# lior1990/hp-vae-gan

Measured on AMD Instinct MI355X. Metric: train iters/sec per pyramid scale, air_balloons 13f@144p, higher is better.
Workload: dtype f32

## Files before the change

### hp-vae-gan_amd/csrc/conv_mfma.hip

```cpp
#include "hpvg_common.h"
#include "hpvg_host.h"
#include "hpvg.h"
#include <stdlib.h>

namespace {

__device__ const float g_zero_word[16] = {0.f, 0.f, 0.f, 0.f, 0.f, 0.f, 0.f, 0.f, 0.f, 0.f, 0.f, 0.f, 0.f, 0.f, 0.f, 0.f};
constexpr long HPVG_ZERO_PLANE_FLOATS = 1L << 18;
__device__ float g_zero_plane[HPVG_ZERO_PLANE_FLOATS];

#ifdef HPVG_TRACE
__device__ unsigned long long g_trace[8192 * 4];
__device__ unsigned long long g_phase[8192 * 4];
#define HPVG_PH(i) { unsigned long long now_ = __builtin_readcyclecounter(); ph_a[i] += now_ - ph_t; ph_t = now_; }
#define HPVG_PH_INIT unsigned long long ph_t = __builtin_readcyclecounter(); unsigned long long ph_a[4] = {0, 0, 0, 0};
#define HPVG_PH_END if (threadIdx.x == 0) { for (int i_ = 0; i_ < 4; ++i_) g_phase[4 * blockIdx.x + i_] = ph_a[i_]; }
#define HPVG_TRACE_BEGIN unsigned long long tr_t0 = wall_clock64(); unsigned long long tr_c0 = __builtin_readcyclecounter();
#define HPVG_TRACE_END                                                              \
  if (threadIdx.x == 0 && blockIdx.x + gridDim.x * (blockIdx.y + gridDim.y * blockIdx.z) < 8192) { \
    unsigned long long* tr = g_trace + 4 * (blockIdx.x + gridDim.x * (blockIdx.y + gridDim.y * blockIdx.z)); \
    tr[0] = tr_t0;                                                                  \
    tr[1] = wall_clock64();                                                         \
    tr[2] = __builtin_amdgcn_s_getreg((31 << 11) | 4);                              \
    tr[3] = (__builtin_amdgcn_s_getreg((31 << 11) | 20) & 0xF) | ((__builtin_readcyclecounter() - tr_c0) << 8); \
// ... 844 lines not shown
          for (int dh = 0; dh < 3; ++dh)
#pragma unroll
            for (int dw = 0; dw < 3; ++dw) {
              const int gwt = gw + dw - 1;
              if (gwt >= 0 && gwt < a.W) v += Pp[(dt * 9 + dh * 3 + dw) * pitch + dh * RS + (dw - 1)];
            }
          sdt[dt] = v;
        }
        rC[p][o] = sdt[0];
        rB[p][o] += sdt[1];
        rA[p][o] += sdt[2];
      }
      __syncthreads();
    }
    if (t >= 1) store_plane(rA, t - 1);
#pragma unroll
    for (int p = 0; p < PPT; ++p)
#pragma unroll
      for (int o = 0; o < COUT; ++o) { rA[p][o] = rB[p][o]; rB[p][o] = rC[p][o]; }
  }
  store_plane(rA, a.T - 1);
}

__global__ void conv_pack_narrow_kernel(const float* __restrict__ w, const float* __restrict__ inv_scale, float* __restrict__ wn,
                                        int Cin_k, int Cout_k, int KT, int NT, int ksteps, int transpose_flip, long total) {
  const long idx = (long)blockIdx.x * blockDim.x + threadIdx.x;
  if (idx >= total) return;
  const int lane = idx & 63;
  long r = idx >> 6;
  const int nt = r % NT;
  const int s = (int)(r / NT);
  const int k = (lane >> 5) * ksteps + s;
  const int n = nt * 32 + (lane & 31);
  const int c = k / KT, dt = k - c * KT;
  const int o = n / 9, tap = dt * 9 + (n - o * 9);
  const int taps = KT * 9;
  float val = 0.f;
  if (o < Cout_k && c < Cin_k) {
    if (!transpose_flip) val = w[((long)o * Cin_k + c) * taps + tap];
    else val = w[((long)c * Cout_k + o) * taps + (taps - 1 - tap)];
    if (inv_scale) val *= inv_scale[0];
  }
  wn[idx] = val;
}

__global__ void conv_pack_kernel(const float* __restrict__ w, const float* __restrict__ inv_scale, float* __restrict__ wp,
                                 int Cin_k, int Cout_k, int taps, int CC, int nchunk, int mbtot, int transpose_flip,
                                 long total_direct, long total) {
  const long idx = (long)blockIdx.x * blockDim.x + threadIdx.x;
  if (idx >= total) return;
  if (idx >= total_direct) {
    const long iw = idx - total_direct;
    const long nw1 = ((long)((Cin_k + WINO_CC - 1) / WINO_CC) * (taps / 9) * 3 * 4 + 4) * mbtot * 64 * (WINO_CC / 2);
    float val = iw < nw1 ? wino_pack_value(w, iw, Cin_k, Cout_k, taps / 9, (Cin_k + WINO_CC - 1) / WINO_CC, mbtot, transpose_flip)
                         : wino2_pack_value(w, iw - nw1, Cin_k, Cout_k, (Cin_k + 3) / 4, 2 * ((mbtot + 1) / 2), transpose_flip);
    if (inv_scale) val *= inv_scale[0];
    wp[idx] = val;
    return;
  }
  const int CP = CC / 2;
  long r = idx;
  const int cp = r % CP; r /= CP;
  const int lane = r % 64; r /= 64;
  const int mb = r % mbtot; r /= mbtot;
  const int tap = r % taps; r /= taps;
  const int ch = (int)r;
  float val = 0.f;
  if (ch < nchunk) {
    const int o = mb * 32 + (lane & 31);
    const int c = ch * CC + 2 * cp + (lane >> 5);
    if (o < Cout_k && c < Cin_k) {
      if (!transpose_flip) val = w[((long)o * Cin_k + c) * taps + tap];
      else val = w[((long)c * Cout_k + o) * taps + (taps - 1 - tap)];
      if (inv_scale) val *= inv_scale[0];
    }
  }
  wp[idx] = val;
}

struct PackBatchArgs {
  const float* w[HPVG_PACK_BATCH_MAX];
  float* wp[HPVG_PACK_BATCH_MAX];
  int flip[HPVG_PACK_BATCH_MAX];
};
__global__ void conv_pack_batch_kernel(const PackBatchArgs a, int C, int taps, int CC, int nchunk, int mbtot, long total_direct,
                                       long total) {
  const long idx = (long)blockIdx.x * blockDim.x + threadIdx.x;
  if (idx >= total) return;
  const int it = blockIdx.y;
  const float* __restrict__ w = a.w[it];
  const int transpose_flip = a.flip[it];
  if (idx >= total_direct) {
    const long iw = idx - total_direct;
    const long nw1 = ((long)((C + WINO_CC - 1) / WINO_CC) * (taps / 9) * 3 * 4 + 4) * mbtot * 64 * (WINO_CC / 2);
    a.wp[it][idx] = iw < nw1 ? wino_pack_value(w, iw, C, C, taps / 9, (C + WINO_CC - 1) / WINO_CC, mbtot, transpose_flip)
                             : wino2_pack_value(w, iw - nw1, C, C, (C + 3) / 4, 2 * ((mbtot + 1) / 2), transpose_flip);
    return;
  }
  const int CP = CC / 2;
  long r = idx;
  const int cp = r % CP; r /= CP;
  const int lane = r % 64; r /= 64;
  const int mb = r % mbtot; r /= mbtot;
  const int tap = r % taps; r /= taps;
  const int ch = (int)r;
  float val = 0.f;
  if (ch < nchunk) {
    const int o = mb * 32 + (lane & 31);
    const int c = ch * CC + 2 * cp + (lane >> 5);
    if (o < C && c < C) {
      if (!transpose_flip) val = w[((long)o * C + c) * taps + tap];
      else val = w[((long)c * C + o) * taps + (taps - 1 - tap)];
    }
  }
  a.wp[it][idx] = val;
}

struct CShape { int B, Cin, Cout, T, H, W, KT; };
inline int conv_check(const CShape& c) {
  if (c.B < 1 || c.Cin < 1 || c.Cout < 1 || c.T < 1 || c.H < 1 || c.W < 1) return HPVG_ERR_ARG;
  return c.KT == 1 || c.KT == 3 ? HPVG_OK : HPVG_ERR_UNSUPPORTED;
}

struct CKnobs {
  bool sk_off;
  bool narrow2_off;
  int narrowt;
  bool w2r;
  bool w2d_off;
  bool w2_split_off;
  int stagger;
  int only_nb, only_mb, only_ntw;
  int env_wino;
  int wino;
  long min_pos;
  int stg;
  int w2d;
  int gen;
// ... 642 lines not shown
    return hpvg_launch_status();
  }
  const int CC = conv_cc(Cin_k);
  hipLaunchKernelGGL(conv_pack_kernel, dim3(hpvg_cdiv(total, 256)), dim3(256), 0, (hipStream_t)stream, w, inv_scale, wp, Cin_k, Cout_k,
                     KT * 9, CC, hpvg_cdiv(Cin_k, CC), hpvg_cdiv(Cout_k, 32), transpose_flip, (long)direct_pack_floats(Cin_k, Cout_k, KT),
                     total);
  return hpvg_launch_status();
}

int pack_batch_launch(int n, const float* const* w, float* const* wp, const int* flip, int C, int KT, bool with2d, void* stream) {
  if (n < 1 || n > HPVG_PACK_BATCH_MAX || !w || !wp || !flip || C <= 4 || (KT != 1 && KT != 3)) return HPVG_ERR_ARG;
  PackBatchArgs a;
  for (int i = 0; i < n; ++i) {
    if (!w[i] || !wp[i]) return HPVG_ERR_ARG;
    a.w[i] = w[i]; a.wp[i] = wp[i]; a.flip[i] = flip[i];
  }
  const int CC = conv_cc(C);
  const long total = (long)wpack_floats(C, C, KT, with2d);
  hipLaunchKernelGGL(conv_pack_batch_kernel, dim3(hpvg_cdiv(total, 256), n), dim3(256), 0, (hipStream_t)stream, a, C, KT * 9, CC,
                     hpvg_cdiv(C, CC), hpvg_cdiv(C, 32), (long)direct_pack_floats(C, C, KT), total);
  return hpvg_launch_status();
}

int write_plan(const Plan& p, int out4, int ntiles, int* out) {
  out[0] = p.L; out[1] = p.Tw; out[2] = p.nrange; out[3] = p.ntw; out[4] = out4; out[5] = p.NB; out[6] = p.MB;
  out[7] = p.gridy; out[8] = (int)p.lds; out[9] = ntiles;
  return HPVG_OK;
}

}

extern "C" {

size_t hpvg_conv_wpack_floats(int Cin, int Cout, int KT) { return wpack_floats(Cin, Cout, KT, true); }
size_t hpvg_conv_wpack_floats_for(int Cin, int Cout, int KT, int B, int T, int H, int W) {
  return wpack_floats(Cin, Cout, KT, wants_wino2d({B, Cin, Cout, T, H, W, KT}));
}
int hpvg_conv_wants_wino2d(int B, int Cin, int Cout, int T, int H, int W, int KT) { return wants_wino2d({B, Cin, Cout, T, H, W, KT}) ? 1 : 0; }

int hpvg_conv_pack_weight_f32(const float* w, const float* inv_scale, float* wp, int Cin_layer, int Cout_layer, int KT,
                              int transpose_flip, void* stream) {
  return pack_weight_launch(w, inv_scale, wp, Cin_layer, Cout_layer, KT, transpose_flip, true, stream);
}
int hpvg_conv_pack_weight_for_f32(const float* w, const float* inv_scale, float* wp, int Cin_layer, int Cout_layer, int KT,
                                  int transpose_flip, int B, int T, int H, int W, void* stream) {
  const int Cin_k = transpose_flip ? Cout_layer : Cin_layer, Cout_k = transpose_flip ? Cin_layer : Cout_layer;
  return pack_weight_launch(w, inv_scale, wp, Cin_layer, Cout_layer, KT, transpose_flip, wants_wino2d({B, Cin_k, Cout_k, T, H, W, KT}), stream);
}
int hpvg_conv_pack_weight_batch_f32(int n, const float* const* w, float* const* wp, const int* flip, int C, int KT, void* stream) {
  return pack_batch_launch(n, w, wp, flip, C, KT, true, stream);
}
int hpvg_conv_pack_weight_batch_for_f32(int n, const float* const* w, float* const* wp, const int* flip, int C, int KT, int B, int T,
                                        int H, int W, void* stream) {
  return pack_batch_launch(n, w, wp, flip, C, KT, wants_wino2d({B, C, C, T, H, W, KT}), stream);
}

int hpvg_conv_fwd_f32(const float* x, const float* wp, const float* bias, const float* in_scale, const float* in_shift,
                      int in_lrelu, float* y, int out_lrelu, const float* out_mask, void* ws, size_t ws_bytes, int B, int Cin,
                      int Cout, int T, int H, int W, int KT, void* stream) {
  return conv_fwd_launch({x, wp, bias, in_scale, in_shift, in_lrelu, y, out_lrelu, out_mask, nullptr, nullptr, ws, ws_bytes,
                          {B, Cin, Cout, T, H, W, KT}, (hipStream_t)stream});
}

size_t hpvg_conv_mask_words(int B, int C, int T, int H, int W) { return (size_t)B * T * H * W * hpvg_cdiv(C, 32); }

int hpvg_conv_fwd_bits_f32(const float* x, const float* wp, const float* bias, float* y, int out_lrelu, const unsigned* mask_bits,
                           unsigned* bits_out, void* ws, size_t ws_bytes, int B, int Cin, int Cout, int T, int H, int W, int KT,
                           void* stream) {
  if (conv_is_narrow(Cin, Cout)) return HPVG_ERR_UNSUPPORTED;
  if (mask_bits && bits_out) return HPVG_ERR_UNSUPPORTED;
  return conv_fwd_launch({x, wp, bias, nullptr, nullptr, 0, y, out_lrelu, nullptr, mask_bits, bits_out, ws, ws_bytes,
                          {B, Cin, Cout, T, H, W, KT}, (hipStream_t)stream});
}

int hpvg_conv_fwd_kernel_kind(int B, int Cin, int Cout, int T, int H, int W, int KT) {
  const CShape c{B, Cin, Cout, T, H, W, KT};
  return conv_check(c) == HPVG_OK ? conv_decide_query(c).kind : HPVG_ERR_ARG;
// ... 94 lines not shown
```

### hp-vae-gan_amd/lib.py

```python
import ctypes
import os
import re

import torch

_HERE = os.path.dirname(os.path.abspath(__file__))
_ROOT = os.path.dirname(_HERE)
LIB_PATH = os.environ.get("HPVG_LIB") or os.path.join(_HERE, "libhpvg.so")
HEADER_PATH = os.path.join(_ROOT, "include", "hpvg.h")

_lib = None

_C_TYPES = {"int": ctypes.c_int, "long": ctypes.c_long, "float": ctypes.c_float, "double": ctypes.c_double,
            "size_t": ctypes.c_size_t, "unsigned": ctypes.c_uint, "unsigned long long": ctypes.c_ulonglong}


class ScalarPtrs(ctypes.Structure):
    """hpvg_scalar_ptrs: the K <= LOG_MAX_K device scalar pointers of one loss-log row, passed by value."""


_C_TYPES["hpvg_scalar_ptrs"] = ScalarPtrs


def parse_header(text):
# ... 4 lines not shown
    for stmt in text.split(";"):
        if not re.search(r"\bhpvg_\w+\s*\(", stmt):
            continue
        m = re.fullmatch(r"(?:\s*extern\s*\"C\"\s*\{)?\s*(\w[\w \t]*?)\s+(hpvg_\w+)\s*\(([^()]*)\)\s*", stmt)
        if not m:
            raise ImportError("hpvg.h: declaration not understood: %s" % " ".join(stmt.split()))
        ret, name, params = m.groups()
        if ret not in ("int", "size_t"):
            raise ImportError("hpvg.h: %s returns %r (int or size_t expected)" % (name, ret))
        args = []
        for prm in ([] if params.strip() in ("", "void") else params.split(",")):
            ctype = ctypes.c_void_p if "*" in prm else _C_TYPES.get(" ".join(prm.split()[:-1]))
            if ctype is None:
                raise ImportError("hpvg.h: %s has a parameter of unknown type: %r" % (name, " ".join(prm.split())))
            args.append(ctype)
        sigs[name] = (_C_TYPES[ret], args)
    return sigs, consts


with open(HEADER_PATH) as _f:
    _SIGNATURES, _CONSTANTS = parse_header(_f.read())
LOG_MAX_K = _CONSTANTS["HPVG_LOG_MAX_K"]
PACK_BATCH_MAX = _CONSTANTS["HPVG_PACK_BATCH_MAX"]
SN_BATCH_MAX = _CONSTANTS["HPVG_SN_BATCH_MAX"]
ScalarPtrs._fields_ = [("p", ctypes.c_void_p * LOG_MAX_K)]
_ERR = {v: k for k, v in _CONSTANTS.items() if k.startswith("HPVG_ERR_")}
_RETURNS_SIZE = frozenset(n for n, (ret, _) in _SIGNATURES.items() if ret is ctypes.c_size_t)


def load():
    global _lib
    if _lib is not None:
        return _lib
    if not os.path.exists(LIB_PATH):
        raise ImportError(
            "hp-vae-gan_amd: %s not found. Build it with `python __graft_entry__.py` (hipcc --offload-arch=gfx950). "
            "This package has no CPU fallback." % LIB_PATH)
    lib = ctypes.CDLL(LIB_PATH)
    missing = [name for name in sorted(_SIGNATURES) if not hasattr(lib, name)]
    if missing:
        raise ImportError("libhpvg.so out of sync with include/hpvg.h: missing=%s" % missing)
    for name, (ret, args) in _SIGNATURES.items():
        fn = getattr(lib, name)
        fn.argtypes = args
        fn.restype = ret
    _lib = lib
# ... 33 lines not shown
```

### hp-vae-gan_amd/modules/_nets.py

```python
import copy
import math

import torch
import torch.nn as nn
from torch.nn import init

from .. import ops
from .. import utils as hp_utils
from ..slab import conv_with_halo


def _kernel_shape(dims):
    return (3,) * dims


class Conv(nn.Module):

    def __init__(self, dims, in_channel, out_channel, ker_size=3, padding=1, stride=1):
        super().__init__()
        if stride != 1 or not ((ker_size == 3 and padding in (0, 1)) or (ker_size == 1 and padding == 0)):
            raise NotImplementedError("the MI355X path implements ker_size=3 with padding in {0, 1} and ker_size=1 with padding 0, stride=1")
        self.dims = dims
        self.ker_size = ker_size
        self.padding = padding if ker_size == 3 else 1
# ... 39 lines not shown
        init.uniform_(bias, -bound, bound)
        self.bias = nn.Parameter(bias)
        self.weight_orig = nn.Parameter(weight)
        h, w = out_channel, weight.numel() // out_channel
        u = torch.nn.functional.normalize(weight.new_empty(h).normal_(0, 1), dim=0, eps=1e-12)
        v = torch.nn.functional.normalize(weight.new_empty(w).normal_(0, 1), dim=0, eps=1e-12)
        self.register_buffer('weight_u', u)
        self.register_buffer('weight_v', v)

    def effective_weight(self):
        return ops.SpectralNormWeight.apply(self.weight_orig, self.weight_u, self.weight_v, self.training, 1e-12)

    halo = None

    def forward(self, x, act=False, weight=None, in_act=False, mask_by_consumer=False, in_bits=None):
        w = weight if weight is not None else self.effective_weight()
        if self.ker_size == 1:
            w = embed_center(w, self.dims)
        if self.halo is not None:
            return conv_with_halo(x, self.halo, lambda xe: ops.Conv.apply(xe, w, self.bias, act, in_act, mask_by_consumer)), None
        return ops.Conv.apply_bits(x, w, self.bias, act, in_act, mask_by_consumer, in_bits)


def sn_weights(convs, x=None):
    out = []
    for i in range(0, len(convs), ops.SN_BATCH_MAX):
        part = convs[i:i + ops.SN_BATCH_MAX]
        args = []
        for m in part:
            args += [m.weight_orig, m.weight_u, m.weight_v]
        out += list(ops.SpectralNormWeightBatch.apply(part[0].training, 1e-12, *args))
    if all(tuple(w.shape[2:]) == (3,) * (w.dim() - 2) for w in out):
        geom_k = None
        if x is not None:
            B, _, T, H, W = ops.geom(x)
            geom_k = (B, T, H, W)
        ops.prepack_weights(out, geom_k=geom_k)
    return out


class BatchNorm(nn.Module):

    def __init__(self, num_features):
        super().__init__()
        self.eps = 1e-5
        self.momentum = 0.1
        self.weight = nn.Parameter(torch.ones(num_features))
        self.bias = nn.Parameter(torch.zeros(num_features))
        self.register_buffer('running_mean', torch.zeros(num_features))
        self.register_buffer('running_var', torch.ones(num_features))
        self.register_buffer('num_batches_tracked', torch.tensor(0, dtype=torch.long))
        self.pending_batches = 0
        self.register_state_dict_pre_hook(BatchNorm._flush_hook)
        self._register_load_state_dict_pre_hook(self._loading_hook)

    @staticmethod
    def _flush_hook(module, prefix, keep_vars):
        module.flush_counter()

    def _loading_hook(self, *args):
# ... 48 lines not shown
            raise NotImplementedError("ConvBlockSN(bn=False) (reflect padding) is never reached on the reference path")
        if act not in ('lrelu', None):
            raise NotImplementedError("only LeakyReLU(0.2) ('lrelu') is implemented on the MI355X path")
        self.conv = SNConv(dims, in_channel, out_channel, ker_size, padding, stride)
        self.act = act

    def forward(self, x, weight=None, in_act=False, mask_by_consumer=False, in_bits=None, with_bits=False):
        y, bits = self.conv(x, act=self.act is not None, weight=weight, in_act=in_act,
                            mask_by_consumer=mask_by_consumer and self.act is not None, in_bits=in_bits)
        return (y, bits) if with_bits else y


class FeatureExtractor(nn.Sequential):

    def __init__(self, dims, in_channel, out_channel, ker_size, padding, stride, num_blocks=2, return_linear=False):
        super().__init__()
        if return_linear:
            raise NotImplementedError("return_linear=True is never used on the reference path")
        self.add_module('conv_block_0', ConvBlockSN(dims, in_channel, out_channel, ker_size, padding, stride))
        for i in range(num_blocks - 1):
            self.add_module('conv_block_{}'.format(i + 1), ConvBlockSN(dims, out_channel, out_channel, ker_size, padding, stride))
        self.add_module('conv_block_{}'.format(num_blocks), ConvBlockSN(dims, out_channel, out_channel, ker_size, padding, stride))

    def forward(self, x, mask_by_consumer=False):
        blocks = list(self)
        last = len(blocks) - 1
        bits = None
        for i, (blk, w) in enumerate(zip(blocks, sn_weights([b.conv for b in blocks], x))):
            x, bits = blk(x, weight=w, in_act=i > 0, mask_by_consumer=(i < last or mask_by_consumer), in_bits=bits, with_bits=True)
        return (x, bits) if mask_by_consumer else x


class EncodeVAE(nn.Module):

    def __init__(self, dims, opt, out_dim=None, num_blocks=2):
        super().__init__()
        if out_dim is None:
            output_dim = opt.nfc
        else:
            assert type(out_dim) is int
            output_dim = out_dim
        self.features = FeatureExtractor(dims, opt.nc_im, opt.nfc, opt.ker_size, opt.ker_size // 2, 1, num_blocks=num_blocks)
        self.mu = ConvBlock(dims, opt.nfc, output_dim, opt.ker_size, opt.ker_size // 2, 1, bn=False, act=None)
        self.logvar = ConvBlock(dims, opt.nfc, output_dim, opt.ker_size, opt.ker_size // 2, 1, bn=False, act=None)

    def forward(self, x):
        features, bits = self.features(x, mask_by_consumer=True)
        return self.mu(features, in_act=True, in_bits=bits), self.logvar(features, in_act=True, in_bits=bits)


def _seven_conv_stack(dims, in_channel, N, opt, padding):
    seq = nn.Sequential()
    seq.add_module('head', ConvBlock(dims, in_channel, N, opt.ker_size, padding, stride=1))
    for i in range(opt.num_layer):
        seq.add_module('block%d' % i, ConvBlock(dims, N, N, opt.ker_size, padding, stride=1))
    seq.add_module('tail', Conv(dims, N, opt.nc_im, opt.ker_size, opt.ker_size // 2, 1))
    return seq


class WDiscriminator(nn.Module):

    def __init__(self, dims, opt):
        super().__init__()
        self.opt = opt
        N = int(opt.nfc)
        self.head = ConvBlockSN(dims, opt.nc_im, N, opt.ker_size, opt.ker_size // 2, stride=1, bn=True, act='lrelu')
        self.body = nn.Sequential()
        for i in range(opt.num_layer):
            self.body.add_module('block%d' % i, ConvBlockSN(dims, N, N, opt.ker_size, opt.ker_size // 2, stride=1, bn=True,
                                                            act='lrelu'))
        self.tail = Conv(dims, N, 1, opt.ker_size, 1, 1)

    def forward(self, x):
        blocks = [self.head] + list(self.body)
        bits = None
        for i, (blk, w) in enumerate(zip(blocks, sn_weights([b.conv for b in blocks], x))):
            x, bits = blk(x, weight=w, in_act=i > 0, mask_by_consumer=True, in_bits=bits, with_bits=True)
        return self.tail(x, in_act=True, in_bits=bits)


class GeneratorHPVAEGAN(nn.Module):

    def __init__(self, dims, opt):
        super().__init__()
        self.dims = dims
        self.opt = opt
        N = int(opt.nfc)
        self.N = N
        self.encode = EncodeVAE(dims, opt, out_dim=opt.latent_dim, num_blocks=opt.enc_blocks)
        self.decoder = _seven_conv_stack(dims, opt.latent_dim, N, opt, opt.padd_size)
        self.body = nn.ModuleList([])
        self.noise_source = None
        self.slab = None

    def init_next_stage(self):
        if len(self.body) == 0:
            self.body.append(_seven_conv_stack(self.dims, self.opt.nc_im, self.N, self.opt, self.opt.padd_size))
        else:
            self.body.append(copy.deepcopy(self.body[-1]))

    def _noise_like(self, ref):
        if self.noise_source is not None:
            return self.noise_source(ref)
        return hp_utils.generate_noise(ref=ref)

    def _reparameterize(self, mu, logvar):
        if self.training:
            return ops.Reparam.apply(mu, logvar, self._noise_like(mu))
        return self._noise_like(mu)

    def forward(self, video, noise_amp, noise_init=None, sample_init=None, mode='rand', stop_idx=None):
        if sample_init is not None:
            assert len(self.body) > sample_init[0], "Strating index must be lower than # of body blocks"

        if noise_init is None:
            mu, logvar = self.encode(video)
            z_vae = self._reparameterize(mu, logvar)
        else:
            z_vae = noise_init

        vae_out = ops.TanhRes.apply(self.decoder(z_vae), None)

        if sample_init is not None:
            x_prev_out = self.refinement_layers(sample_init[0], sample_init[1], noise_amp, mode, stop_idx)
        else:
            x_prev_out = self.refinement_layers(0, vae_out, noise_amp, mode, stop_idx)

        if noise_init is None:
            return x_prev_out, vae_out, (mu, logvar)
        return x_prev_out, vae_out

    def forward_pair(self, video, noise_amp, noise_init):
        assert self.training and self.slab is None
        B = video.shape[0]
        mu, logvar = self.encode(video)
        z = ops.Concat2.apply(self._reparameterize(mu, logvar), noise_init)
        bns = [m for part in (self.decoder, self.body) for m in part.modules() if isinstance(m, BatchNorm)]
        for m in bns:
            m.groups = 2
        try:
            vae_out = ops.TanhRes.apply(self.decoder(z), None)
            x = vae_out
            for idx, block in enumerate(self.body):
                if self.opt.vae_levels == idx + 1 and not self.opt.train_all:
                    x.detach_()
                size = self._level_size(idx + 1)
                if self.dims == 2 or self.opt.vae_levels <= idx + 1:
                    if self.noise_source is None:
                        up, up_noisy = ops.UpsampleACNoise.apply(x, tuple(size), float(noise_amp[idx + 1]), B)
                    else:
                        ref = x.new_empty((B, x.shape[1], *size))
                        noise = ops.concat_batch([B, self._noise_like(ref)])
                        up, up_noisy = ops.UpsampleAC.apply(x, tuple(size), noise, float(noise_amp[idx + 1]))
                else:
                    up = up_noisy = ops.UpsampleAC.apply(x, tuple(size), None, 0.0)
                x = ops.TanhRes.apply(block(up_noisy), up)
        finally:
            for m in bns:
                m.groups = 1
# ... 244 lines not shown
```

### hp-vae-gan_amd/ops.py

```python
import ctypes
import os

import torch
from torch.autograd import Function
from torch.autograd.function import once_differentiable

from .lib import PACK_BATCH_MAX, SN_BATCH_MAX, call, load, ptr, stream

_ws_cache = {}
_kernel_timer = None


class KernelTimer:

    def __init__(self, match):
        self.match = match
        self.events = []

    def begin(self, desc):
        fam = self.match(desc)
        if not fam:
            return None
        e0 = torch.cuda.Event(enable_timing=True)
        e0.record()
        return (fam, e0)

    def end(self, tok, key):
        if tok is None:
            return
        e1 = torch.cuda.Event(enable_timing=True)
# ... 47 lines not shown
    if x.dim() == 5:
        B, C, T, H, W = x.shape
    elif x.dim() == 4:
        B, C, H, W = x.shape
        T = 1
    else:
        raise RuntimeError("expected a 4-D or 5-D activation, got %s" % (tuple(x.shape),))
    return B, C, T, H, W


def _kt(w_shape):
    if len(w_shape) == 5:
        if tuple(w_shape[2:]) != (3, 3, 3):
            raise RuntimeError("only 3x3x3 kernels are supported on the MI355X path, got %s" % (tuple(w_shape),))
        return 3
    if len(w_shape) == 4:
        if tuple(w_shape[2:]) != (3, 3):
            raise RuntimeError("only 3x3 kernels are supported on the MI355X path, got %s" % (tuple(w_shape),))
        return 1
    raise RuntimeError("bad weight shape %s" % (tuple(w_shape),))


_pack_cache = {}


def weights_changed():
    _pack_cache.clear()


def _wants_2d(geom_k, cin_k, cout_k, KT):
    if geom_k is None or KT != 3:
        return None if geom_k is None else False
    B, T, H, W = geom_k
    return load().hpvg_conv_wants_wino2d(B, cin_k, cout_k, T, H, W, KT) == 1


def pack_weight(w, flip, geom_k=None):
    w = _c(w)
    Co, Ci = w.shape[0], w.shape[1]
    KT = _kt(w.shape)
    cin_k, cout_k = (Co, Ci) if flip else (Ci, Co)
    has2d = _wants_2d(geom_k, cin_k, cout_k, KT)
    key = (w.data_ptr(), bool(flip), tuple(w.shape))
    hit = _pack_cache.get(key)
    if hit is not None and hit[0] == w._version and hit[1].device == w.device and (hit[3] is None or hit[3] is True or has2d is False):
        return hit[2]
    if geom_k is None:
        n = call("hpvg_conv_wpack_floats", cin_k, cout_k, KT)
        wp = torch.empty(n, dtype=torch.float32, device=w.device)
        call("hpvg_conv_pack_weight_f32", ptr(w), None, ptr(wp), Ci, Co, KT, 1 if flip else 0, stream())
# ... 18 lines not shown
                items.append((w, bool(f), key))
    if not items:
        return
    shape = tuple(items[0][0].shape)
    items = [it for it in items if tuple(it[0].shape) == shape][:PACK_BATCH_MAX]
    C, KT = shape[0], _kt(shape)
    has2d = _wants_2d(geom_k, C, C, KT)
    if geom_k is None:
        nfl = call("hpvg_conv_wpack_floats", C, C, KT)
    else:
        nfl = call("hpvg_conv_wpack_floats_for", C, C, KT, *geom_k)
    dev = items[0][0].device
    wps = [torch.empty(nfl, dtype=torch.float32, device=dev) for _ in items]
    m = len(items)
    PA, IA = ctypes.c_void_p * m, ctypes.c_int * m
    if geom_k is None:
        call("hpvg_conv_pack_weight_batch_f32", m, PA(*[ptr(it[0]) for it in items]), PA(*[ptr(t) for t in wps]),
             IA(*[1 if it[1] else 0 for it in items]), C, KT, stream())
    else:
        call("hpvg_conv_pack_weight_batch_for_f32", m, PA(*[ptr(it[0]) for it in items]), PA(*[ptr(t) for t in wps]),
             IA(*[1 if it[1] else 0 for it in items]), C, KT, *geom_k, stream())
    for (w, f, key), wp in zip(items, wps):
        _pack_cache[key] = (w._version, w.detach(), wp, has2d)


def conv_fwd_raw(x, w, bias, out_lrelu=False, flip=False, in_affine=None, in_lrelu=False, out_mask=None, mask_bits=None,
                 want_bits=False):
    x = _c(x)
    B, C, T, H, W = geom(x)
    KT = _kt(w.shape)
    Co_l, Ci_l = w.shape[0], w.shape[1]
    cin_k, cout_k = (Co_l, Ci_l) if flip else (Ci_l, Co_l)
    if C != cin_k:
        raise RuntimeError("conv: input has %d channels, weight expects %d" % (C, cin_k))
    wp = pack_weight(w, flip, (B, T, H, W))
    shape = (B, cout_k, T, H, W) if x.dim() == 5 else (B, cout_k, H, W)
    y = torch.empty(shape, dtype=torch.float32, device=x.device)
    sc = sh = None
    if in_affine is not None:
        sc, sh = in_affine
    timed = None
    if _kernel_timer is not None:
        var = "pro" if in_affine is not None else ("mask" if (out_mask is not None or mask_bits is not None) else ("bits" if want_bits else "plain"))
        timed = _kernel_timer.begin({"op": "conv", "Cin": cin_k, "Cout": cout_k, "KT": KT, "flip": flip, "var": var})
    nws = call("hpvg_conv_fwd_ws_bytes", B, cin_k, cout_k, T, H, W, KT)
    ws = _scratch(nws, x.device) if nws else (None, 0)
# ... 915 lines not shown
        slot[i] = v
    return slot[:len(vals)].to(device, non_blocking=True)


def lerp(a, b, alpha):
    a, b = _c(a.detach()), _c(b.detach())
    out = torch.empty_like(a)
    call("hpvg_lerp_f32", ptr(a), ptr(b), ptr(alpha), ptr(out), a.numel(), stream())
    return out


def sqsum(flat):
    out = _scalar_out(flat.device)
    call("hpvg_sqsum_f32", ptr(flat), ptr(out), *_reduce_ws(flat.device), flat.numel(), stream())
    return out


def clip_scale_(flat_grad, sq, max_norm, coef_out=None):
    call("hpvg_clip_scale_f32", ptr(flat_grad), flat_grad.numel(), ptr(sq), float(max_norm), ptr(coef_out),
         stream())


def adam_step_(p, g, m, v, lr, beta1, beta2, eps, step, step_dev=None):
    weights_changed()
    call("hpvg_adam_step_f32", ptr(p), ptr(g), ptr(m), ptr(v), p.numel(), float(lr), float(beta1), float(beta2),
         float(eps), int(step), ptr(step_dev), stream())


def counter_inc_(counter):
    call("hpvg_counter_inc_i32", ptr(counter), stream())


def state_digest_(t, salt, acc):
    if t.element_size() not in (4, 8):
        raise RuntimeError("state_digest: 4-byte and 8-byte dtypes only, got %s" % t.dtype)
    t = _c(t.detach())
    n = t.numel() * (t.element_size() // 4)
    call("hpvg_state_digest_u32", ptr(t) if n else None, n, int(salt) & 0xFFFFFFFFFFFFFFFF, ptr(acc), stream())
    return n


def state_digest(tensors):
    tensors = list(tensors)
    if not tensors:
        return 0
    acc = torch.zeros(1, dtype=torch.int64, device=tensors[0].device)
    salt = 0
# ... 439 lines not shown
```

### hp-vae-gan_amd/optim.py

```python
import torch

from . import ops

_ALIGN = 64


class ParamArena:

    def __init__(self, module):
        params = list(module.parameters())
        if not params:
            raise ValueError("module has no parameters")
        dev = params[0].device
        offs, total = [], 0
        for p in params:
            offs.append(total)
            total += (p.numel() + _ALIGN - 1) // _ALIGN * _ALIGN
        self.flat = torch.zeros(total, dtype=torch.float32, device=dev)
        self.grad = torch.zeros(total, dtype=torch.float32, device=dev)
        self.range = {}
        with torch.no_grad():
            for p, o in zip(params, offs):
                n = p.numel()
                self.flat[o:o + n].copy_(p.detach().reshape(-1))
                p.data = self.flat[o:o + n].view(p.shape)
                p.grad = self.grad[o:o + n].view(p.shape)
                self.range[id(p)] = (o, n)
        self.params = params
        self.total = total

    def span(self, params):
        rs = sorted(self.range[id(p)] for p in params)
        lo = rs[0][0]
        hi = rs[-1][0] + (rs[-1][1] + _ALIGN - 1) // _ALIGN * _ALIGN
        covered = sum((n + _ALIGN - 1) // _ALIGN * _ALIGN for _, n in rs)
        if covered != hi - lo:
            raise ValueError("parameter group is not contiguous in the arena")
        return lo, hi

    def zero_grad(self):
        self.grad.zero_()
        for p in self.params:
            o, n = self.range[id(p)]
            g = p.grad
            if g is None or g.data_ptr() != self.grad.data_ptr() + 4 * o:
                p.grad = self.grad[o:o + n].view(p.shape)

    def clip_grad_norm_(self, max_norm, info=None):
        sq = ops.sqsum(self.grad)
        ops.clip_scale_(self.grad, sq, max_norm, info)


# ... 70 lines not shown
```

### include/hpvg.h

```cpp
#ifndef HPVG_H
#define HPVG_H
#include <stddef.h>
#ifdef __cplusplus
extern "C" {
#endif

#define HPVG_OK 0
#define HPVG_ERR_ARG (-1)
#define HPVG_ERR_WORKSPACE (-2)
#define HPVG_ERR_UNSUPPORTED (-3)
#define HPVG_ERR_LAUNCH (-4)

size_t hpvg_conv_wpack_floats(int Cin, int Cout, int KT);
int hpvg_conv_pack_weight_f32(const float* w, const float* inv_scale, float* wp, int Cin_layer, int Cout_layer, int KT,
                              int transpose_flip, void* stream);
#define HPVG_PACK_BATCH_MAX 16
int hpvg_conv_pack_weight_batch_f32(int n, const float* const* w, float* const* wp, const int* flip, int C, int KT, void* stream);
size_t hpvg_conv_wpack_floats_for(int Cin, int Cout, int KT, int B, int T, int H, int W);
int hpvg_conv_wants_wino2d(int B, int Cin, int Cout, int T, int H, int W, int KT);
int hpvg_conv_pack_weight_for_f32(const float* w, const float* inv_scale, float* wp, int Cin_layer, int Cout_layer, int KT,
                                  int transpose_flip, int B, int T, int H, int W, void* stream);
int hpvg_conv_pack_weight_batch_for_f32(int n, const float* const* w, float* const* wp, const int* flip, int C, int KT, int B, int T,
                                        int H, int W, void* stream);
size_t hpvg_conv_fwd_ws_bytes(int B, int Cin, int Cout, int T, int H, int W, int KT);
int hpvg_conv_fwd_f32(const float* x, const float* wp, const float* bias, const float* in_scale, const float* in_shift,
                      int in_lrelu, float* y, int out_lrelu, const float* out_mask, void* ws, size_t ws_bytes, int B, int Cin,
                      int Cout, int T, int H, int W, int KT, void* stream);
size_t hpvg_conv_mask_words(int B, int C, int T, int H, int W);
int hpvg_conv_fwd_bits_f32(const float* x, const float* wp, const float* bias, float* y, int out_lrelu, const unsigned* mask_bits,
                           unsigned* bits_out, void* ws, size_t ws_bytes, int B, int Cin, int Cout, int T, int H, int W, int KT,
                           void* stream);
int hpvg_conv_fwd_plan(int B, int Cin, int Cout, int T, int H, int W, int KT, int* out10);
int hpvg_conv_fwd_kernel_kind(int B, int Cin, int Cout, int T, int H, int W, int KT);
int hpvg_conv_w2_split(int B, int Cin, int Cout, int T, int H, int W, int KT, int* out4);
int hpvg_conv_wino_config(int mode, long min_positions);
int hpvg_conv_wino_plan(int B, int Cin, int Cout, int T, int H, int W, int KT, int* out10);
int hpvg_conv_narrow_plan(int B, int Cin, int Cout, int T, int H, int W, int KT, int* out55);
int hpvg_conv_narrowt_plan(int B, int Cin, int Cout, int T, int H, int W, int KT, int* out57);
int hpvg_conv_narrowt_config(int mode);
size_t hpvg_conv_bwd_weight_ws_bytes(int B, int Cin, int Cout, int T, int H, int W, int KT);
int hpvg_conv_bwd_weight_f32(const float* dy, const float* x, const float* in_scale, const float* in_shift, int in_lrelu,
                             float* dw, int accumulate, void* ws, size_t ws_bytes, int B, int Cin, int Cout, int T, int H,
                             int W, int KT, void* stream);
int hpvg_conv_bwd_weight_plan(int B, int Cin, int Cout, int T, int H, int W, int KT, int* out10);
int hpvg_conv_bwd_weight_kernel_kind(int B, int Cin, int Cout, int T, int H, int W, int KT);
int hpvg_conv_bwd_weight_wino_config(int mode);
// ... 170 lines not shown
```

Measured before the change: 34.56.

## Batch weight prepacking of heterogeneous convs into single multi-item kernel launches

Adds a conv_pack_multi_kernel that packs up to 64 weights of differing shapes, narrow or wide layouts and flip modes in one launch, writing into a single aligned arena. The generator, discriminator and encoder stacks now prepack all their forward and flipped (backward) weights upfront. The aim is to replace many small per-layer pack launches and Python calls with a few batched ones. Adam steps now invalidate only the pack-cache entries inside the stepped optimizer's arena instead of clearing the whole cache, so packs of other networks survive across steps. In exchange, some flipped weights may be packed that are never used, and the partial invalidation logic adds risk of serving stale packs.

```diff
diff --git a/hp-vae-gan_amd/csrc/conv_mfma.hip b/hp-vae-gan_amd/csrc/conv_mfma.hip
--- a/hp-vae-gan_amd/csrc/conv_mfma.hip
+++ b/hp-vae-gan_amd/csrc/conv_mfma.hip
@@ -890,10 +890,8 @@
   store_plane(rA, a.T - 1);
 }
 
-__global__ void conv_pack_narrow_kernel(const float* __restrict__ w, const float* __restrict__ inv_scale, float* __restrict__ wn,
-                                        int Cin_k, int Cout_k, int KT, int NT, int ksteps, int transpose_flip, long total) {
-  const long idx = (long)blockIdx.x * blockDim.x + threadIdx.x;
-  if (idx >= total) return;
+__device__ __forceinline__ float pack_narrow_value(const float* __restrict__ w, const float* __restrict__ inv_scale, long idx,
+                                                   int Cin_k, int Cout_k, int KT, int NT, int ksteps, int transpose_flip) {
   const int lane = idx & 63;
   long r = idx >> 6;
   const int nt = r % NT;
@@ -909,22 +907,19 @@
     else val = w[((long)c * Cout_k + o) * taps + (taps - 1 - tap)];
     if (inv_scale) val *= inv_scale[0];
   }
-  wn[idx] = val;
-}
-
-__global__ void conv_pack_kernel(const float* __restrict__ w, const float* __restrict__ inv_scale, float* __restrict__ wp,
-                                 int Cin_k, int Cout_k, int taps, int CC, int nchunk, int mbtot, int transpose_flip,
-                                 long total_direct, long total) {
-  const long idx = (long)blockIdx.x * blockDim.x + threadIdx.x;
-  if (idx >= total) return;
+  return val;
+}
+
+__device__ __forceinline__ float pack_wide_value(const float* __restrict__ w, const float* __restrict__ inv_scale, long idx,
+                                                 int Cin_k, int Cout_k, int taps, int CC, int nchunk, int mbtot,
+                                                 int transpose_flip, long total_direct) {
   if (idx >= total_direct) {
     const long iw = idx - total_direct;
     const long nw1 = ((long)((Cin_k + WINO_CC - 1) / WINO_CC) * (taps / 9) * 3 * 4 + 4) * mbtot * 64 * (WINO_CC / 2);
     float val = iw < nw1 ? wino_pack_value(w, iw, Cin_k, Cout_k, taps / 9, (Cin_k + WINO_CC - 1) / WINO_CC, mbtot, transpose_flip)
                          : wino2_pack_value(w, iw - nw1, Cin_k, Cout_k, (Cin_k + 3) / 4, 2 * ((mbtot + 1) / 2), transpose_flip);
     if (inv_scale) val *= inv_scale[0];
-    wp[idx] = val;
-    return;
+    return val;
   }
   const int CP = CC / 2;
   long r = idx;
@@ -943,7 +938,22 @@
       if (inv_scale) val *= inv_scale[0];
     }
   }
-  wp[idx] = val;
+  return val;
+}
+
+__global__ void conv_pack_narrow_kernel(const float* __restrict__ w, const float* __restrict__ inv_scale, float* __restrict__ wn,
+                                        int Cin_k, int Cout_k, int KT, int NT, int ksteps, int transpose_flip, long total) {
+  const long idx = (long)blockIdx.x * blockDim.x + threadIdx.x;
+  if (idx >= total) return;
+  wn[idx] = pack_narrow_value(w, inv_scale, idx, Cin_k, Cout_k, KT, NT, ksteps, transpose_flip);
+}
+
+__global__ void conv_pack_kernel(const float* __restrict__ w, const float* __restrict__ inv_scale, float* __restrict__ wp,
+                                 int Cin_k, int Cout_k, int taps, int CC, int nchunk, int mbtot, int transpose_flip,
+                                 long total_direct, long total) {
+  const long idx = (long)blockIdx.x * blockDim.x + threadIdx.x;
+  if (idx >= total) return;
+  wp[idx] = pack_wide_value(w, inv_scale, idx, Cin_k, Cout_k, taps, CC, nchunk, mbtot, transpose_flip, total_direct);
 }
 
 struct PackBatchArgs {
@@ -956,32 +966,31 @@
   const long idx = (long)blockIdx.x * blockDim.x + threadIdx.x;
   if (idx >= total) return;
   const int it = blockIdx.y;
-  const float* __restrict__ w = a.w[it];
-  const int transpose_flip = a.flip[it];
-  if (idx >= total_direct) {
-    const long iw = idx - total_direct;
-    const long nw1 = ((long)((C + WINO_CC - 1) / WINO_CC) * (taps / 9) * 3 * 4 + 4) * mbtot * 64 * (WINO_CC / 2);
-    a.wp[it][idx] = iw < nw1 ? wino_pack_value(w, iw, C, C, taps / 9, (C + WINO_CC - 1) / WINO_CC, mbtot, transpose_flip)
-                             : wino2_pack_value(w, iw - nw1, C, C, (C + 3) / 4, 2 * ((mbtot + 1) / 2), transpose_flip);
-    return;
-  }
-  const int CP = CC / 2;
-  long r = idx;
-  const int cp = r % CP; r /= CP;
-  const int lane = r % 64; r /= 64;
-  const int mb = r % mbtot; r /= mbtot;
-  const int tap = r % taps; r /= taps;
-  const int ch = (int)r;
-  float val = 0.f;
-  if (ch < nchunk) {
-    const int o = mb * 32 + (lane & 31);
-    const int c = ch * CC + 2 * cp + (lane >> 5);
-    if (o < C && c < C) {
-      if (!transpose_flip) val = w[((long)o * C + c) * taps + tap];
-      else val = w[((long)c * C + o) * taps + (taps - 1 - tap)];
-    }
-  }
-  a.wp[it][idx] = val;
+  a.wp[it][idx] = pack_wide_value(a.w[it], nullptr, idx, C, C, taps, CC, nchunk, mbtot, a.flip[it], total_direct);
+}
+
+struct PackMultiArgs {
+  const float* w[HPVG_PACK_MULTI_MAX];
+  const float* inv_scale[HPVG_PACK_MULTI_MAX];
+  float* wp[HPVG_PACK_MULTI_MAX];
+  int Cin_k[HPVG_PACK_MULTI_MAX], Cout_k[HPVG_PACK_MULTI_MAX];
+  int mode[HPVG_PACK_MULTI_MAX];
+  int CC[HPVG_PACK_MULTI_MAX];
+  int n1[HPVG_PACK_MULTI_MAX];
+  int n2[HPVG_PACK_MULTI_MAX];
+  int total_direct[HPVG_PACK_MULTI_MAX];
+  int total[HPVG_PACK_MULTI_MAX];
+};
+static_assert(sizeof(PackMultiArgs) + 16 <= 4096, "conv_pack_multi_kernel's arguments must stay under 4 KB");
+__global__ void conv_pack_multi_kernel(const PackMultiArgs a, int KT) {
+  const int it = blockIdx.y;
+  const long idx = (long)blockIdx.x * blockDim.x + threadIdx.x;
+  if (idx >= a.total[it]) return;
+  const int mode = a.mode[it];
+  float* __restrict__ wp = a.wp[it];
+  if (mode & 2) wp[idx] = pack_narrow_value(a.w[it], a.inv_scale[it], idx, a.Cin_k[it], a.Cout_k[it], KT, a.n1[it], a.n2[it], mode & 1);
+  else wp[idx] = pack_wide_value(a.w[it], a.inv_scale[it], idx, a.Cin_k[it], a.Cout_k[it], KT * 9, a.CC[it], a.n1[it], a.n2[it],
+                                 mode & 1, a.total_direct[it]);
 }
 
 struct CShape { int B, Cin, Cout, T, H, W, KT; };
@@ -1670,6 +1679,53 @@
   return hpvg_launch_status();
 }
 
+struct PackItem {
+  int Cin_k, Cout_k, flip;
+  bool narrow, with2d;
+  int CC, n1, n2;
+  size_t total_direct, total;
+};
+int pack_item_resolve(const int* desc, int KT, PackItem& p) {
+  const int Cin_l = desc[0], Cout_l = desc[1], B = desc[3], T = desc[4], H = desc[5], W = desc[6];
+  if (Cin_l < 1 || Cout_l < 1 || B < 0 || (B > 0 && (T < 1 || H < 1 || W < 1))) return HPVG_ERR_ARG;
+  p.flip = desc[2] ? 1 : 0;
+  p.Cin_k = p.flip ? Cout_l : Cin_l;
+  p.Cout_k = p.flip ? Cin_l : Cout_l;
+  const bool sections2d = B == 0 || wants_wino2d({B, p.Cin_k, p.Cout_k, T, H, W, KT});
+  p.total = wpack_floats(p.Cin_k, p.Cout_k, KT, sections2d);
+  p.narrow = conv_is_narrow(p.Cin_k, p.Cout_k);
+  if (p.narrow) {
+    p.with2d = false;
+    p.CC = 0; p.n1 = hpvg_cdiv(9 * p.Cout_k, 32); p.n2 = hpvg_cdiv(p.Cin_k * KT, 2);
+    p.total_direct = p.total;
+  } else {
+    p.with2d = sections2d && conv_is_wino2d(cknobs(), p.Cin_k, p.Cout_k, KT);
+    p.CC = conv_cc(p.Cin_k); p.n1 = hpvg_cdiv(p.Cin_k, p.CC); p.n2 = hpvg_cdiv(p.Cout_k, 32);
+    p.total_direct = direct_pack_floats(p.Cin_k, p.Cout_k, KT);
+  }
+  return p.total < ((size_t)1 << 31) ? HPVG_OK : HPVG_ERR_UNSUPPORTED;
+}
+
+int pack_multi_launch(int n, const float* const* w, const float* const* inv_scale, float* const* wp, const int* desc, int KT,
+                      void* stream) {
+  if (n < 1 || n > HPVG_PACK_MULTI_MAX || !w || !wp || !desc || (KT != 1 && KT != 3)) return HPVG_ERR_ARG;
+  PackMultiArgs a{};
+  size_t most = 0;
+  for (int i = 0; i < n; ++i) {
+    if (!w[i] || !wp[i]) return HPVG_ERR_ARG;
+    PackItem p;
+    const int rc = pack_item_resolve(desc + 7 * i, KT, p);
+    if (rc != HPVG_OK) return rc;
+    a.w[i] = w[i]; a.inv_scale[i] = inv_scale ? inv_scale[i] : nullptr; a.wp[i] = wp[i];
+    a.Cin_k[i] = p.Cin_k; a.Cout_k[i] = p.Cout_k; a.mode[i] = p.flip | (p.narrow ? 2 : 0);
+    a.CC[i] = p.CC; a.n1[i] = p.n1; a.n2[i] = p.n2;
+    a.total_direct[i] = (int)p.total_direct; a.total[i] = (int)p.total;
+    if (p.total > most) most = p.total;
+  }
+  hipLaunchKernelGGL(conv_pack_multi_kernel, dim3(hpvg_cdiv((long)most, 256), n), dim3(256), 0, (hipStream_t)stream, a, KT);
+  return hpvg_launch_status();
+}
+
 int write_plan(const Plan& p, int out4, int ntiles, int* out) {
   out[0] = p.L; out[1] = p.Tw; out[2] = p.nrange; out[3] = p.ntw; out[4] = out4; out[5] = p.NB; out[6] = p.MB;
   out[7] = p.gridy; out[8] = (int)p.lds; out[9] = ntiles;
@@ -1701,6 +1757,20 @@
 int hpvg_conv_pack_weight_batch_for_f32(int n, const float* const* w, float* const* wp, const int* flip, int C, int KT, int B, int T,
                                         int H, int W, void* stream) {
   return pack_batch_launch(n, w, wp, flip, C, KT, wants_wino2d({B, C, C, T, H, W, KT}), stream);
+}
+int hpvg_conv_pack_weight_multi_f32(int n, const float* const* w, const float* const* inv_scale, float* const* wp, const int* desc,
+                                    int KT, void* stream) {
+  return pack_multi_launch(n, w, inv_scale, wp, desc, KT, stream);
+}
+int hpvg_conv_pack_multi_plan(int n, const int* desc, int KT, int* narrow, int* with2d, size_t* floats) {
+  if (n < 1 || n > HPVG_PACK_MULTI_MAX || !desc || !narrow || !with2d || !floats || (KT != 1 && KT != 3)) return HPVG_ERR_ARG;
+  for (int i = 0; i < n; ++i) {
+    PackItem p;
+    const int rc = pack_item_resolve(desc + 7 * i, KT, p);
+    if (rc != HPVG_OK) return rc;
+    narrow[i] = p.narrow ? 1 : 0; with2d[i] = p.with2d ? 1 : 0; floats[i] = p.total;
+  }
+  return HPVG_OK;
 }
 
 int hpvg_conv_fwd_f32(const float* x, const float* wp, const float* bias, const float* in_scale, const float* in_shift,
diff --git a/hp-vae-gan_amd/lib.py b/hp-vae-gan_amd/lib.py
--- a/hp-vae-gan_amd/lib.py
+++ b/hp-vae-gan_amd/lib.py
@@ -50,6 +50,7 @@
     _SIGNATURES, _CONSTANTS = parse_header(_f.read())
 LOG_MAX_K = _CONSTANTS["HPVG_LOG_MAX_K"]
 PACK_BATCH_MAX = _CONSTANTS["HPVG_PACK_BATCH_MAX"]
+PACK_MULTI_MAX = _CONSTANTS["HPVG_PACK_MULTI_MAX"]
 SN_BATCH_MAX = _CONSTANTS["HPVG_SN_BATCH_MAX"]
 ScalarPtrs._fields_ = [("p", ctypes.c_void_p * LOG_MAX_K)]
 _ERR = {v: k for k, v in _CONSTANTS.items() if k.startswith("HPVG_ERR_")}
diff --git a/hp-vae-gan_amd/modules/_nets.py b/hp-vae-gan_amd/modules/_nets.py
--- a/hp-vae-gan_amd/modules/_nets.py
+++ b/hp-vae-gan_amd/modules/_nets.py
@@ -85,7 +85,11 @@
         return ops.Conv.apply_bits(x, w, self.bias, act, in_act, mask_by_consumer, in_bits)
 
 
-def sn_weights(convs, x=None):
+def _plain3(m):
+    return m.ker_size == 3 and m.halo is None and getattr(m, 'padding', 1) == 1
+
+
+def sn_weights(convs, x=None, extra=()):
     out = []
     for i in range(0, len(convs), ops.SN_BATCH_MAX):
         part = convs[i:i + ops.SN_BATCH_MAX]
@@ -98,7 +102,24 @@
         if x is not None:
             B, _, T, H, W = ops.geom(x)
             geom_k = (B, T, H, W)
-        ops.prepack_weights(out, geom_k=geom_k)
+        if ops.PACK_MULTI and x is not None and all(_plain3(m) for m in convs):
+            grad = torch.is_grad_enabled()
+            rg = grad and x.requires_grad
+            items = []
+            for m, w in zip(convs, out):
+                square = w.shape[0] == w.shape[1] and w.shape[0] > 4
+                items.append((w, False, geom_k))
+                if square or rg:
+                    items.append((w, True, geom_k))
+                rg = rg or (grad and w.requires_grad)
+            for m, flipped in extra:
+                if _plain3(m):
+                    items.append((m.weight, False, geom_k))
+                    if flipped and rg:
+                        items.append((m.weight, True, geom_k))
+            ops.prepack_many(items)
+        else:
+            ops.prepack_weights(out, geom_k=geom_k)
     return out
 
 
@@ -193,11 +214,11 @@
             self.add_module('conv_block_{}'.format(i + 1), ConvBlockSN(dims, out_channel, out_channel, ker_size, padding, stride))
         self.add_module('conv_block_{}'.format(num_blocks), ConvBlockSN(dims, out_channel, out_channel, ker_size, padding, stride))
 
-    def forward(self, x, mask_by_consumer=False):
+    def forward(self, x, mask_by_consumer=False, heads=()):
         blocks = list(self)
         last = len(blocks) - 1
         bits = None
-        for i, (blk, w) in enumerate(zip(blocks, sn_weights([b.conv for b in blocks], x))):
+        for i, (blk, w) in enumerate(zip(blocks, sn_weights([b.conv for b in blocks], x, extra=[(m, False) for m in heads]))):
             x, bits = blk(x, weight=w, in_act=i > 0, mask_by_consumer=(i < last or mask_by_consumer), in_bits=bits, with_bits=True)
         return (x, bits) if mask_by_consumer else x
 
@@ -216,7 +237,7 @@
         self.logvar = ConvBlock(dims, opt.nfc, output_dim, opt.ker_size, opt.ker_size // 2, 1, bn=False, act=None)
 
     def forward(self, x):
-        features, bits = self.features(x, mask_by_consumer=True)
+        features, bits = self.features(x, mask_by_consumer=True, heads=(self.mu.conv, self.logvar.conv))
         return self.mu(features, in_act=True, in_bits=bits), self.logvar(features, in_act=True, in_bits=bits)
 
 
@@ -245,7 +266,7 @@
     def forward(self, x):
         blocks = [self.head] + list(self.body)
         bits = None
-        for i, (blk, w) in enumerate(zip(blocks, sn_weights([b.conv for b in blocks], x))):
+        for i, (blk, w) in enumerate(zip(blocks, sn_weights([b.conv for b in blocks], x, extra=[(self.tail, True)]))):
             x, bits = blk(x, weight=w, in_act=i > 0, mask_by_consumer=True, in_bits=bits, with_bits=True)
         return self.tail(x, in_act=True, in_bits=bits)
 
@@ -280,6 +301,32 @@
             return ops.Reparam.apply(mu, logvar, self._noise_like(mu))
         return self._noise_like(mu)
 
+    def _prepack_pass(self, z):
+        if not ops.PACK_MULTI or self.slab is not None:
+            return
+        B = z.shape[0]
+        stacks = [(self.decoder, (B,) + tuple(ops.geom(z)[2:]), False)]
+        for idx, block in enumerate(self.body):
+            size = tuple(self._level_size(idx + 1))
+            stacks.append((block, (B,) + ((1,) + size if self.dims == 2 else size), self._detach_before(idx)))
+        grad = torch.is_grad_enabled()
+        cut = max((i for i, s in enumerate(stacks) if s[2]), default=0)
+        fwd, flipped = [], []
+        rg = z.requires_grad
+        for i, (stack, geom_k, detach) in enumerate(stacks):
+            if detach:
+                rg = False
+            convs = [m for m in stack.modules() if isinstance(m, Conv)]
+            plain = all(_plain3(m) for m in convs)
+            for m in convs:
+                if plain:
+                    fwd.append((m.weight, False, geom_k))
+                    if grad and rg and i >= cut:
+                        flipped.append((m.weight, True, geom_k))
+                rg = rg or m.weight.requires_grad or m.bias.requires_grad
+        ops.prepack_many(fwd)
+        ops.prepack_many(flipped)
+
     def forward(self, video, noise_amp, noise_init=None, sample_init=None, mode='rand', stop_idx=None):
         if sample_init is not None:
             assert len(self.body) > sample_init[0], "Strating index must be lower than # of body blocks"
@@ -290,6 +337,8 @@
         else:
             z_vae = noise_init
 
+        if sample_init is None and stop_idx is None:
+            self._prepack_pass(z_vae)
         vae_out = ops.TanhRes.apply(self.decoder(z_vae), None)
 
         if sample_init is not None:
@@ -306,6 +355,7 @@
         B = video.shape[0]
         mu, logvar = self.encode(video)
         z = ops.Concat2.apply(self._reparameterize(mu, logvar), noise_init)
+        self._prepack_pass(z)
         bns = [m for part in (self.decoder, self.body) for m in part.modules() if isinstance(m, BatchNorm)]
         for m in bns:
             m.groups = 2
diff --git a/hp-vae-gan_amd/ops.py b/hp-vae-gan_amd/ops.py
--- a/hp-vae-gan_amd/ops.py
+++ b/hp-vae-gan_amd/ops.py
@@ -1,11 +1,12 @@
 import ctypes
 import os
+import weakref
 
 import torch
 from torch.autograd import Function
 from torch.autograd.function import once_differentiable
 
-from .lib import PACK_BATCH_MAX, SN_BATCH_MAX, call, load, ptr, stream
+from .lib import PACK_BATCH_MAX, PACK_MULTI_MAX, SN_BATCH_MAX, call, load, ptr, stream
 
 _ws_cache = {}
 _kernel_timer = None
@@ -99,10 +100,28 @@
 
 
 _pack_cache = {}
-
-
-def weights_changed():
-    _pack_cache.clear()
+PACK_MULTI = os.environ.get("HPVG_PACK_MULTI", "1") != "0"
+_arenas = []
+
+
+def register_arena(flat):
+    _arenas[:] = [r for r in _arenas if r() is not None]
+    _arenas.append(weakref.ref(flat))
+
+
+def weights_changed(stepped=None):
+    if stepped is None or not PACK_MULTI:
+        _pack_cache.clear()
+        return
+    spans = [(t.data_ptr(), t.data_ptr() + 4 * t.numel()) for t in (r() for r in _arenas) if t is not None]
+    a = stepped.data_ptr()
+    own = [s for s in spans if s[0] <= a < s[1]]
+    if not own:
+        _pack_cache.clear()
+        return
+    lo, hi = own[0]
+    for key in [k for k in _pack_cache if lo <= k[0] < hi or not any(s[0] <= k[0] < s[1] for s in spans)]:
+        del _pack_cache[key]
 
 
 def _wants_2d(geom_k, cin_k, cout_k, KT):
@@ -167,6 +186,73 @@
              IA(*[1 if it[1] else 0 for it in items]), C, KT, *geom_k, stream())
     for (w, f, key), wp in zip(items, wps):
         _pack_cache[key] = (w._version, w.detach(), wp, has2d)
+
+
+_PACK_ALIGN = 64
+
+
+def pack_many_layout(specs, gap=0):
+    descs, by_kt = [], {}
+    for i, (w, flip, geom_k, _) in enumerate(specs):
+        if not w.is_contiguous():
+            raise RuntimeError("hp-vae-gan_amd: tensor must be contiguous")
+        by_kt.setdefault(_kt(w.shape), []).append(i)
+        descs.append([w.shape[1], w.shape[0], 1 if flip else 0] + ([int(v) for v in geom_k] if geom_k is not None else [0, 0, 0, 0]))
+    launches = [idx[i:i + PACK_MULTI_MAX] for _, idx in sorted(by_kt.items()) for i in range(0, len(idx), PACK_MULTI_MAX)]
+    floats = [0] * len(descs)
+    for idx in launches:
+        m = len(idx)
+        narrow, with2d, nfl = (ctypes.c_int * m)(), (ctypes.c_int * m)(), (ctypes.c_size_t * m)()
+        call("hpvg_conv_pack_multi_plan", m, (ctypes.c_int * (7 * m))(*[v for i in idx for v in descs[i]]), _kt(specs[idx[0]][0].shape),
+             narrow, with2d, nfl)
+        for i, n in zip(idx, nfl):
+            floats[i] = int(n)
+    offsets, total = [], 0
+    for n in floats:
+        offsets.append(total)
+        total = (total + n + gap + _PACK_ALIGN - 1) // _PACK_ALIGN * _PACK_ALIGN
+    return launches, offsets, floats, total, descs
+
+
+def pack_many_into(specs, layout, base):
+    launches, offsets, floats, total, descs = layout
+    if base.numel() < total or base.data_ptr() % (4 * _PACK_ALIGN):
+        raise RuntimeError("pack_many_into: the buffer must hold %d floats and start on a 256-byte boundary" % total)
+    wps = [base[o:o + n] for o, n in zip(offsets, floats)]
+    for idx in launches:
+        m = len(idx)
+        PA = ctypes.c_void_p * m
+        call("hpvg_conv_pack_weight_multi_f32", m, PA(*[ptr(specs[i][0]) for i in idx]), PA(*[ptr(specs[i][3]) for i in idx]),
+             PA(*[ptr(wps[i]) for i in idx]), (ctypes.c_int * (7 * m))(*[v for i in idx for v in descs[i]]),
+             _kt(specs[idx[0]][0].shape), stream())
+    return wps
+
+
+def prepack_many(items):
+    todo = {}
+    for w, flip, geom_k in items:
+        if not w.is_contiguous():
+            continue
+        KT = _kt(w.shape)
+        cin_k, cout_k = (w.shape[0], w.shape[1]) if flip else (w.shape[1], w.shape[0])
+        has2d = _wants_2d(geom_k, cin_k, cout_k, KT)
+        key = (w.data_ptr(), bool(flip), tuple(w.shape))
+        hit = _pack_cache.get(key)
+        if hit is not None and hit[0] == w._version and hit[1].device == w.device and (hit[3] is None or hit[3] is True or has2d is False):
+            continue
+        prev = todo.get(key)
+        if prev is None or (prev[4] is False and has2d is not False):
+            todo[key] = (w, bool(flip), geom_k, None, has2d)
+    if not todo:
+        return 0
+    keys = list(todo)
+    specs = [todo[k][:4] for k in keys]
+    layout = pack_many_layout(specs)
+    base = torch.empty(layout[3], dtype=torch.float32, device=specs[0][0].device)
+    for key, wp in zip(keys, pack_many_into(specs, layout, base)):
+        w = todo[key][0]
+        _pack_cache[key] = (w._version, w.detach(), wp, todo[key][4])
+    return len(keys)
 
 
 def conv_fwd_raw(x, w, bias, out_lrelu=False, flip=False, in_affine=None, in_lrelu=False, out_mask=None, mask_bits=None,
@@ -1128,7 +1214,7 @@
 
 
 def adam_step_(p, g, m, v, lr, beta1, beta2, eps, step, step_dev=None):
-    weights_changed()
+    weights_changed(p)
     call("hpvg_adam_step_f32", ptr(p), ptr(g), ptr(m), ptr(v), p.numel(), float(lr), float(beta1), float(beta2),
          float(eps), int(step), ptr(step_dev), stream())
 
diff --git a/hp-vae-gan_amd/optim.py b/hp-vae-gan_amd/optim.py
--- a/hp-vae-gan_amd/optim.py
+++ b/hp-vae-gan_amd/optim.py
@@ -28,6 +28,7 @@
                 self.range[id(p)] = (o, n)
         self.params = params
         self.total = total
+        ops.register_arena(self.flat)
 
     def span(self, params):
         rs = sorted(self.range[id(p)] for p in params)
diff --git a/include/hpvg.h b/include/hpvg.h
--- a/include/hpvg.h
+++ b/include/hpvg.h
@@ -22,6 +22,10 @@
                                   int transpose_flip, int B, int T, int H, int W, void* stream);
 int hpvg_conv_pack_weight_batch_for_f32(int n, const float* const* w, float* const* wp, const int* flip, int C, int KT, int B, int T,
                                         int H, int W, void* stream);
+#define HPVG_PACK_MULTI_MAX 64
+int hpvg_conv_pack_weight_multi_f32(int n, const float* const* w, const float* const* inv_scale, float* const* wp, const int* desc,
+                                    int KT, void* stream);
+int hpvg_conv_pack_multi_plan(int n, const int* desc, int KT, int* narrow, int* with2d, size_t* floats);
 size_t hpvg_conv_fwd_ws_bytes(int B, int Cin, int Cout, int T, int H, int W, int KT);
 int hpvg_conv_fwd_f32(const float* x, const float* wp, const float* bias, const float* in_scale, const float* in_shift,
                       int in_lrelu, float* y, int out_lrelu, const float* out_mask, void* ws, size_t ws_bytes, int B, int Cin,
```

Result: no change. 34.80, median of 6 (+0.7%).
